# johannah/drqv2

Measured on AMD Instinct MI355X. Metric: agent updates/sec (batch=256, 9x84x84 obs), higher is better.
Workload: dtype f32; 1 GPU; cheetah_run batch_size=256/GPU (256 global) 9x84x84 u8 obs, A=6, feature_dim=50, hidden_dim=1024, fp32, use_tb=True; parallelism=dp1, global_batch=256

## Files before the change

drqv2_amd/_lib.py:

```python
import ctypes as C
import os

HERE = os.path.dirname(os.path.abspath(__file__))
LIB_PATH = os.path.join(HERE, "libdrqv2_hip.so")

c_float_p = C.c_void_p
c_u8_p = C.c_void_p
stream_t = C.c_void_p


class DrqStep(C.Structure):
    _fields_ = [
        ("B", C.c_int), ("global_B", C.c_int), ("C", C.c_int), ("A", C.c_int), ("F", C.c_int), ("H", C.c_int),
        ("obs", c_u8_p), ("next_obs", c_u8_p),
        ("action", c_float_p), ("reward", c_float_p), ("discount", c_float_p),
        ("shift_obs", c_float_p), ("shift_next", c_float_p),
        ("noise_critic", c_float_p), ("noise_actor", c_float_p),
        ("base_grid", c_float_p),
        ("params", c_float_p), ("grads", c_float_p), ("adam_m", c_float_p), ("adam_v", c_float_p),
        ("ws", c_float_p), ("ws_bytes", C.c_size_t),
        ("sums", c_float_p),
        ("lr", C.c_double), ("tau", C.c_double),
        ("std", C.c_float), ("clip", C.c_float),
        ("step_critic", C.c_long), ("step_enc", C.c_long), ("step_actor", C.c_long),
# ... 18 lines not shown
    "drq_conv1_aug_fwd": (I, [P, P, P, P, P, P, P, P, P, I, I, P]),
    "drq_conv1_aug_fwd_bf16": (I, [P, P, P, P, P, P, P, P, P, I, I, P]),
    "drq_conv1_aug_fwd_bf16_nhwc": (I, [P, P, P, P, P, P, P, P, P, I, I, P]),
    "drq_conv1_aug_fwd_indexed": (I, [P, P, P, P, P, P, P, P, P, P, P, I, I, P]),
    "drq_conv1_aug_fwd_frames": (I, [P, P, L, L, P, P, P, P, P, P, P, P, P, I, I, P]),
    "drq_conv1_aug_fwd_frames_bf16": (I, [P, P, L, L, P, P, P, P, P, P, P, P, P, I, I, P]),
    "drq_conv3x3_fwd": (I, [P, P, P, P, I, I, I, I, I, L, L, L, L, P]),
    "drq_conv3x3_dgrad": (I, [P, P, P, P, I, I, L, L, L, L, P]),
    "drq_conv3x3_fwd_wino": (I, [P, P, P, P, I, I, I, L, L, L, L, P]),
    "drq_conv3x3_dgrad_wino": (I, [P, P, P, P, I, I, L, L, L, L, P]),
    "drq_conv3x3_wgrad_wino": (I, [P, P, P, P, I, I, L, L, L, L, P, SZ, P]),
    "drq_conv3x3_wgrad": (I, [P, P, P, P, I, I, I, I, L, L, L, L, P, SZ, P]),
    "drq_conv3x3_wgrad_ws_bytes": (SZ, []),
    "drq_conv3x3_fwd_bf16": (I, [P, P, P, P, I, I, I, L, L, L, L, P]),
    "drq_conv3x3_dgrad_bf16": (I, [P, P, P, P, I, I, L, L, L, L, P]),
    "drq_conv3x3_wgrad_bf16": (I, [P, P, P, P, I, I, L, L, L, L, P, SZ, P]),
    "drq_conv3x3_fwd_bf16_nhwc": (I, [P, P, P, P, I, I, I, I, I, P]),
    "drq_conv3x3_dgrad_bf16_nhwc": (I, [P, P, P, P, I, I, I, I, L, L, L, L, P]),
    "drq_conv3x3_wgrad_bf16_nhwc": (I, [P, P, P, P, I, I, I, L, L, L, L, P, SZ, P]),
    "drq_gemm_f32": (I, [P, L, I, P, L, I, P, L, I, I, I, I, L, L, L, P, L, I, P, I, L, I, I, I, P, SZ, P]),
    "drq_gemm_batched_f32": (I, [I, P, L, I, P, L, I, P, L, I, I, I, P, I, P, I, P, I, I, I, P, SZ, P]),
    "drq_gemm_batched_bf16": (I, [I, P, L, I, P, L, I, P, L, I, I, I, P, I, P, I, P, I, I, P, SZ, P]),
    "drq_gemm_batched_partial": (I, [I, P, L, I, P, L, I, P, L, I, I, I, P, P, SZ, C.POINTER(I), P]),
    "drq_mlp_fwd": (I, [I, P, L, P, L, P, L, I, I, I, P, I, P, P, C.POINTER(I), P]),
    "drq_mlp_dgrad": (I, [I, P, L, P, L, P, L, I, I, I, P, I, P]),
    "drq_mlp_wgrad_dgrad": (I, [I, P, L, P, L, P, P, P, L, P, L, P, I, I, I, I, P]),
    "drq_ln_l1_fwd": (I, [I, P, P, P, P, P, P, P, P, P, P, P, P, P, P, P, P, P, I, I, I, L, P]),
    "drq_policy_out_l1_fwd": (I, [P, P, P, P, I, I, I, I, I, F, F, I, P, P, P, L, P, P, P, L, I, P, P, P, P]),
    "drq_qout_fwd": (I, [I, P, P, P, P, I, I, P]),
    "drq_qout_bwd": (I, [I, P, P, P, P, P, P, I, I, P]),
    "drq_ln_tanh_fwd_multi": (I, [I, P, I, P, P, P, P, P, P, I, I, P]),
    "drq_ln_tanh_fwd": (I, [P, I, P, P, P, I, P, P, I, I, P]),
    "drq_ln_tanh_fwd2": (I, [P, P, I, P, P, P, P, P, I, P, I, P, P, P, P, I, I, P]),
    "drq_ln_tanh_bwd": (I, [P, I, P, I, P, I, P, P, P, P, P, P, P, I, I, P]),
    "drq_colsum": (I, [P, L, L, P, L, I, I, I, P]),
    "drq_trunc_normal_sample": (I, [P, P, F, F, I, P, P, L, I, I, P]),
    "drq_copy_cols": (I, [P, I, P, L, I, I, P]),
    "drq_td_mse": (I, [P, P, P, P, P, P, P, P, P, I, F, P]),
    "drq_td_mse_w": (I, [P, P, P, P, P, P, P, P, P, P, P, I, F, P]),
    "drq_actor_loss": (I, [P, P, P, L, P, F, P, P, P, I, I, F, P]),
    "drq_actor_dmu": (I, [P, P, L, I, P, P, I, I, P]),
    "drq_actor_loss_bc": (I, [P, P, P, L, P, L, P, F, F, P, P, P, I, I, F, P]),
    "drq_qout_bwd_actor_bc": (I, [P, P, P, L, P, L, P, F, F, I, F, P, P, P, P, I, I, P]),
    "drq_actor_dmu_bc": (I, [P, P, L, I, P, P, L, P, L, F, P, I, I, P]),
    "drq_policy_out_bwd_bc": (I, [P, P, L, I, P, P, L, P, L, F, P, P, P, P, P, I, I, I, P, I, P]),
    "drq_adam_flat": (I, [P, P, P, P, L, D, L, F, P, D, P]),
# ... 92 lines not shown
```

drqv2_amd/csrc/gemm.hip:

```cpp
#include "common.h"
#include "internal.h"
#include "../../include/drqv2_hip.h"
#include <type_traits>

namespace {

constexpr int BK0 = 32;

constexpr int MAXB = 8;

struct Epilogue {
  const float* bias[MAXB];
  const float* aux[MAXB];
  float* rowsum[MAXB];
  int ldaux;
  int relu;
  int scatter_hw;
};

struct GemmArgs {
  const float* A[MAXB];
  const float* B[MAXB];
  float* C[MAXB];
  long lda, ldb, ldc;
// ... 81 lines not shown
    constexpr int KSTEP = 256 / BR;
    const bool rok = row0 + r < rows;
#pragma unroll
    for (int p = 0; p < BR * BK / 256; ++p)
      S[r * PK + kk0 + p * KSTEP] = (rok && k0 + kk0 + p * KSTEP < kend) ? reg[p] : 0.f;
  }
}

template <int BR, int BK>
__device__ __forceinline__ float tile_rowsum(const float (&reg)[BR * BK / 256], int row0, int rows, int k0, int kend,
                                             int tid) {
  const int r = tid % BR, kk0 = tid / BR;
  constexpr int KSTEP = 256 / BR;
  float s = 0.f;
  if (row0 + r < rows) {
#pragma unroll
    for (int p = 0; p < BR * BK / 256; ++p)
      if (k0 + kk0 + p * KSTEP < kend) s += reg[p];
  }
  return s;
}

template <int TM, int TN, bool A_KC, bool B_KC, bool V4, int BK = BK0, bool FULL = false>
__global__ __launch_bounds__(256) void gemm_kernel(GemmArgs g) {
  constexpr int PK = BK + 2;
  constexpr int BM = 32 * TM, BN = 32 * TN;
  constexpr int RA = BM * BK / 256, RB = BN * BK / 256;
  constexpr int D = (TM * TN == 1 && BK == 32) ? 4 : 2;
  __shared__ __attribute__((aligned(16))) float As[2][BM * PK];
  __shared__ __attribute__((aligned(16))) float Bs[2][BN * PK];

  const int tid = threadIdx.x;
  const int lane = tid & 63, wid = tid >> 6;
  const int wm = wid >> 1, wn = wid & 1;
  const int z = blockIdx.z;
  const int batch = z / g.splitk, ks = z - batch * g.splitk;
  const int m0 = blockIdx.y * BM, n0 = blockIdx.x * BN;
  const int kbeg = ks * g.kchunk;
  const int kend = min(g.K, kbeg + g.kchunk);
  const float* A = g.A[batch];
  const float* B = g.B[batch];

  float ra[D][RA], rb[D][RB];

  f32x4 acc[TM][TN];
#pragma unroll
  for (int i = 0; i < TM; ++i)
#pragma unroll
    for (int j = 0; j < TN; ++j) acc[i][j] = (f32x4){0.f, 0.f, 0.f, 0.f};

  const int arow = (wm * TM * 16 + (lane & 15)) * PK + (lane >> 4);
  const int brow = (wn * TN * 16 + (lane & 15)) * PK + (lane >> 4);
  const int nsteps = (kend - kbeg + BK - 1) / BK;

  auto fetch = [&](int t, float (&fa)[RA], float (&fb)[RB]) {
    const int tc = t < nsteps ? t : nsteps - 1;
    load_tile<BM, A_KC, V4, BK, FULL>(A, g.lda, m0, g.M, kbeg + tc * BK, kend, fa, tid);
    load_tile<BN, B_KC, V4, BK, FULL>(B, g.ldb, n0, g.N, kbeg + tc * BK, kend, fb, tid);
  };
  bool do_rs = false;
  if constexpr (!A_KC) do_rs = g.ep.rowsum[batch] != nullptr && blockIdx.x == 0;
  float rs = 0.f;
  if (nsteps > 0) {
    fetch(0, ra[0], rb[0]);
    if constexpr (!A_KC)
      if (do_rs) rs += tile_rowsum<BM, BK>(ra[0], m0, g.M, kbeg, kend, tid);
    store_tile<BM, A_KC, V4, BK, FULL>(As[0], ra[0], m0, g.M, kbeg, kend, tid);
    store_tile<BN, B_KC, V4, BK, FULL>(Bs[0], rb[0], n0, g.N, kbeg, kend, tid);
#pragma unroll
    for (int d = 1; d <= D; ++d) fetch(d, ra[d % D], rb[d % D]);
  }
  __syncthreads();
  auto step = [&](int t, auto sc) {
    constexpr int s = decltype(sc)::value;
    const float* as = As[s & 1];
    const float* bs = Bs[s & 1];
    float a[BK / 4][TM], b[BK / 4][TN];
#pragma unroll
    for (int kk = 0; kk < BK / 4; ++kk) {
#pragma unroll
      for (int i = 0; i < TM; ++i) a[kk][i] = as[arow + i * 16 * PK + kk * 4];
#pragma unroll
      for (int j = 0; j < TN; ++j) b[kk][j] = bs[brow + j * 16 * PK + kk * 4];
    }
// ... 87 lines not shown
#pragma unroll
    for (int j = 0; j < TN; ++j) {
      const int n = ncol0 + j * 16;
      long cbase = n;
      if (e.scatter_hw > 0) {
        const int hw = e.scatter_hw, hp = hw + 4;
        const int ch = n / (hw * hw);
        const int rr = n - ch * hw * hw;
        const int y = rr / hw, x = rr - y * hw;
        cbase = ((long)ch * hp + (y + 2)) * hp + (x + 2);
      }
#pragma unroll
      for (int r = 0; r < 4; ++r) {
        const int m = mrow0 + i * 16 + r;
        if (m < g.M && n < g.N) {
          float v = acc[i][j][r] + bv[j];
          if (e.relu) v = v > 0.f ? v : 0.f;
          v = av[i][j][r] > 0.f ? v : 0.f;
          if (e.scatter_hw > 0) c[(long)m * 32 * (e.scatter_hw + 4) * (e.scatter_hw + 4) + cbase] = v;
          else c[(long)m * g.ldc + cbase] = v;
        }
      }
    }
}

typedef __bf16 bf16x8_t __attribute__((ext_vector_type(8)));
typedef unsigned u32x4_t __attribute__((ext_vector_type(4)));

__device__ __forceinline__ unsigned pack_bf16_pair(float lo, float hi) {
  typedef __bf16 bf16x2_t __attribute__((ext_vector_type(2)));
  const bf16x2_t v = {(__bf16)lo, (__bf16)hi};
  return __builtin_bit_cast(unsigned, v);
}

constexpr int BF_BM = 64, BF_BK = 64, BF_PD = 36;

template <bool V4>
__device__ __forceinline__ void bf_load_kc(const float* P, long ld, int row0, int rows, int k0, int kend,
                                           float (&v)[16], int tid) {
  const int r = tid >> 2, kq = (tid & 3) * 16;
  const int row = row0 + r;
  if (V4 && row < rows && k0 + kq + 16 <= kend) {
    const f32x4* p = reinterpret_cast<const f32x4*>(P + (long)row * ld + k0 + kq);
#pragma unroll
    for (int i = 0; i < 4; ++i) {
      const f32x4 t = p[i];
// ... 202 lines not shown
    return v4 ? launch<TM, TN, true, false, true, BK>(g, st) : launch<TM, TN, true, false, false, BK>(g, st);
  if (!a_kc && !b_kc) return launch<TM, TN, false, false, false, BK>(g, st);
  return DRQ_EARG;
}

template <bool A_KC, bool B_KC>
int launch_bf16(const GemmArgs& g, bool v4, hipStream_t st) {
  const bool wide = g.N > 64 && g.N <= 128 && g.K >= 4096;
  const int bn = wide ? 2 * BF_BM : BF_BM;
  dim3 grid((g.N + bn - 1) / bn, (g.M + BF_BM - 1) / BF_BM, g.nbatch * g.splitk);
  if (wide) {
    if (v4) hipLaunchKernelGGL((gemm_bf16_kernel<A_KC, B_KC, true, 2>), grid, dim3(256), 0, st, g);
    else hipLaunchKernelGGL((gemm_bf16_kernel<A_KC, B_KC, false, 2>), grid, dim3(256), 0, st, g);
  } else if (v4) hipLaunchKernelGGL((gemm_bf16_kernel<A_KC, B_KC, true>), grid, dim3(256), 0, st, g);
  else hipLaunchKernelGGL((gemm_bf16_kernel<A_KC, B_KC, false>), grid, dim3(256), 0, st, g);
  DRQ_LAUNCH_CHECK();
  g_last_splitk = g.splitk;
  if (g.splitk > 1 && !g_leave_partials) {
    const long mn = (long)g.M * g.N;
    dim3 rg((unsigned)((mn + 255) / 256), g.nbatch);
    hipLaunchKernelGGL(splitk_reduce_kernel, rg, dim3(256), 0, st, g);
    DRQ_LAUNCH_CHECK();
  }
  return DRQ_OK;
}

}

int drq_gemm_batched_any(int bf16, int nbatch, const float* const* A, long lda, int a_kc, const float* const* B, long ldb,
                         int b_kc, float* const* C, long ldc, int M, int N, int K, const float* const* bias, int relu,
                         const float* const* aux, int ldaux, float* const* rowsum, int scatter_hw, int tile,
                         int splitk, float* ws, size_t ws_bytes, hipStream_t st) {
  if (!A || !B || !C || M <= 0 || N <= 0 || K <= 0 || nbatch <= 0 || nbatch > MAXB) return DRQ_EARG;
  for (int b = 0; b < nbatch; ++b)
    if (!A[b] || !B[b] || !C[b]) return DRQ_EARG;
  if (rowsum && a_kc) return DRQ_EARG;
  if (bf16) {
    if (!a_kc && b_kc) return DRQ_EARG;
    const int cus = drq_num_cus();
    const long tiles = (long)((M + 63) / 64) * ((N + 63) / 64) * nbatch;
    if (rowsum && splitk == 0 && tiles < 2L * cus && K >= 512) {
      for (int b = 0; b < nbatch; ++b)
        if (rowsum[b]) {
          const int rc = drq_colsum(A[b], lda, 0, rowsum[b], 0, K, M, 1, st);
          if (rc != DRQ_OK) return rc;
        }
// ... 24 lines not shown
    }
    g.lda = lda; g.ldb = ldb; g.ldc = ldc; g.M = M; g.N = N; g.K = K;
    g.nbatch = nbatch; g.splitk = splitk; g.kchunk = kchunk; g.part = ws;
    g.ep.ldaux = ldaux; g.ep.relu = relu; g.ep.scatter_hw = scatter_hw;
    if (a_kc && b_kc) return launch_bf16<true, true>(g, v4, st);
    if (a_kc && !b_kc) return launch_bf16<true, false>(g, v4, st);
    return launch_bf16<false, false>(g, v4, st);
  }
  if (nbatch == 1 && tile == 0 && splitk == 0 && N >= 4096 && N % 32 == 0 && !bias && !relu && a_kc && !b_kc &&
      K <= 128 && !rowsum) {
    const int rc =
        drq_skinny_dgrad(A[0], lda, B[0], ldb, C[0], ldc, M, N, K, aux ? aux[0] : nullptr, ldaux, scatter_hw, st);
    if (rc != DRQ_EARG) return rc;
  }
  if (nbatch == 1 && tile == 0 && splitk == 0 && scatter_hw == 0 && !a_kc && !b_kc && M <= 128 && N >= 4096 && !bias &&
      !relu && !aux) {
    const int rc = drq_trunk_wgrad(A[0], lda, B[0], ldb, C[0], ldc, M, N, K, rowsum ? rowsum[0] : nullptr, st);
    if (rc != DRQ_EARG) return rc;
  }
  if (tile == 0 && splitk == 0 && scatter_hw == 0) {
    const int rc = drq_gemm2(nbatch, A, lda, a_kc, B, ldb, b_kc, C, ldc, M, N, K, bias, relu, aux, ldaux, rowsum, st);
    if (rc != DRQ_EARG) return rc;
  }
  const int cus = drq_num_cus();
  const long t_big = (long)((M + 63) / 64) * ((N + 63) / 64) * nbatch;
  const long t_small = (long)((M + 31) / 32) * ((N + 31) / 32) * nbatch;
  if (tile == 0) tile = (t_big >= 2L * cus) ? 2 : 1;
  const long tiles = tile == 2 ? t_big : (tile >= 3 ? (t_big + t_small) / 2 : t_small);
  if (rowsum) splitk = 1;
  if (splitk == 0) {
    splitk = 1;
    if (tiles < 2L * cus && K >= 256) {
      splitk = (int)((3L * cus + tiles - 1) / tiles);
      const int maxs = K / 128;
      if (splitk > maxs) splitk = maxs;
      if (splitk < 1) splitk = 1;
    }
  }
  int kchunk = ((K + splitk - 1) / splitk + 63) / 64 * 64;
  splitk = (K + kchunk - 1) / kchunk;
  if (splitk > 1 && (!ws || (size_t)nbatch * splitk * M * N * sizeof(float) > ws_bytes)) return DRQ_EWS;
  GemmArgs g{};
  auto al16 = [](const void* p) { return ((uintptr_t)p & 15) == 0; };
  bool v4 = (K % 4 == 0) && (a_kc || b_kc);
  if (a_kc) v4 = v4 && lda % 4 == 0;
  if (b_kc) v4 = v4 && ldb % 4 == 0;
  for (int b = 0; b < nbatch; ++b) {
    g.A[b] = A[b]; g.B[b] = B[b]; g.C[b] = C[b];
    g.ep.bias[b] = bias ? bias[b] : nullptr;
    g.ep.aux[b] = aux ? aux[b] : nullptr;
    g.ep.rowsum[b] = rowsum ? rowsum[b] : nullptr;
    if (a_kc) v4 = v4 && al16(A[b]);
    if (b_kc) v4 = v4 && al16(B[b]);
  }
  g.lda = lda; g.ldb = ldb; g.ldc = ldc; g.M = M; g.N = N; g.K = K;
  g.nbatch = nbatch; g.splitk = splitk; g.kchunk = kchunk; g.part = ws;
  g.ep.ldaux = ldaux; g.ep.relu = relu; g.ep.scatter_hw = scatter_hw;
  if (tile == 3) return dispatch<2, 1>(g, a_kc, b_kc, v4, st);
  if (tile == 4) return dispatch<1, 2>(g, a_kc, b_kc, v4, st);
  if (tile == 5) return dispatch<1, 1, 64>(g, a_kc, b_kc, v4, st);
  if (tile == 6) return dispatch<2, 2, 64>(g, a_kc, b_kc, v4, st);
  return tile == 2 ? dispatch<2, 2>(g, a_kc, b_kc, v4, st) : dispatch<1, 1>(g, a_kc, b_kc, v4, st);
}

DRQ_API int drq_gemm_batched_f32(int nbatch, const float* const* A, long lda, int a_kc, const float* const* B, long ldb,
                         int b_kc, float* const* C, long ldc, int M, int N, int K, const float* const* bias, int relu,
                         const float* const* aux, int ldaux, float* const* rowsum, int scatter_hw, int tile,
                         int splitk, float* ws, size_t ws_bytes, drq_stream_t stream) {
  return drq_gemm_batched_any(0, nbatch, A, lda, a_kc, B, ldb, b_kc, C, ldc, M, N, K, bias, relu, aux, ldaux, rowsum,
                              scatter_hw, tile, splitk, ws, ws_bytes, (hipStream_t)stream);
}

DRQ_API int drq_gemm_batched_bf16(int nbatch, const float* const* A, long lda, int a_kc, const float* const* B, long ldb,
                          int b_kc, float* const* C, long ldc, int M, int N, int K, const float* const* bias, int relu,
                          const float* const* aux, int ldaux, float* const* rowsum, int scatter_hw, int splitk,
                          float* ws, size_t ws_bytes, drq_stream_t stream) {
  return drq_gemm_batched_any(1, nbatch, A, lda, a_kc, B, ldb, b_kc, C, ldc, M, N, K, bias, relu, aux, ldaux, rowsum,
                              scatter_hw, 0, splitk, ws, ws_bytes, (hipStream_t)stream);
}

// ... 4 lines not shown
  if (!bf16 && a_kc && b_kc && N <= 128 && K >= 4096 && ldc == N) {
    int sk = 1;
    const int rc = drq_trunk_fwd_partial(nbatch, A, lda, B, ldb, M, N, K, ws, ws_bytes, &sk, st);
    if (rc == DRQ_OK) {
      if (splitk_out) *splitk_out = sk;
      return DRQ_OK;
    }
    if (rc != DRQ_EARG) return rc;
  }
  g_leave_partials = true;
  g_last_splitk = 1;
  const int rc = drq_gemm_batched_any(bf16, nbatch, A, lda, a_kc, B, ldb, b_kc, C, ldc, M, N, K, bias, 0, nullptr, 0,
                                      nullptr, 0, bf16 ? 0 : 1, 0, ws, ws_bytes, st);
  g_leave_partials = false;
  if (splitk_out) *splitk_out = g_last_splitk;
  return rc;
}

DRQ_API int drq_gemm_batched_partial(int nbatch, const float* const* A, long lda, int a_kc, const float* const* B, long ldb,
                             int b_kc, float* const* C, long ldc, int M, int N, int K, const float* const* bias,
                             float* ws, size_t ws_bytes, int* splitk_out, drq_stream_t stream) {
  return drq_gemm_batched_partial_any(0, nbatch, A, lda, a_kc, B, ldb, b_kc, C, ldc, M, N, K, bias, ws, ws_bytes,
                                      splitk_out, (hipStream_t)stream);
}

DRQ_API int drq_gemm_f32(const float* A, long lda, int a_kc, const float* B, long ldb, int b_kc, float* C, long ldc,
                 int M, int N, int K, int nbatch, long a_bs, long b_bs, long c_bs, const float* bias, long bias_bs,
                 int relu, const float* aux, int ldaux, long aux_bs, int scatter_hw, int tile, int splitk,
                 float* ws, size_t ws_bytes, drq_stream_t stream) {
  if (!A || !B || !C || nbatch <= 0 || nbatch > MAXB) return DRQ_EARG;
  const float *Ap[MAXB], *Bp[MAXB], *bp[MAXB], *xp[MAXB];
  float* Cp[MAXB];
  for (int b = 0; b < nbatch; ++b) {
    Ap[b] = A + b * a_bs; Bp[b] = B + b * b_bs; Cp[b] = C + b * c_bs;
    bp[b] = bias ? bias + b * bias_bs : nullptr;
    xp[b] = aux ? aux + b * aux_bs : nullptr;
  }
  return drq_gemm_batched_f32(nbatch, Ap, lda, a_kc, Bp, ldb, b_kc, Cp, ldc, M, N, K, bias ? bp : nullptr, relu,
                              aux ? xp : nullptr, ldaux, nullptr, scatter_hw, tile, splitk, ws, ws_bytes, stream);
}
```

drqv2_amd/csrc/internal.h:

```cpp
#pragma once
#include "common.h"

int drq_ln_tanh_fwd_multi_ex(int n, const float* const* z, int ldz, const float* const* gamma,
                             const float* const* beta, float* const* out, const int* ldo, float* const* xhat,
                             float* const* rstd, int rows, int F, const float* const* tail, const int* tail_ld,
                             int tail_n, hipStream_t st);
int drq_ln_tanh_fwd_multi_part(int n, const float* const* z, int ldz, const float* const* gamma,
                               const float* const* beta, float* const* out, const int* ldo, float* const* xhat,
                               float* const* rstd, int rows, int F, const float* const* tail, const int* tail_ld,
                               int tail_n, const float* part, const float* const* bias, int splitk, hipStream_t st);
int drq_ln_tanh_bwd_part(const float* dh0, int ld0, const float* dh1, int ld1, const float* h, int ldh,
                         const float* xhat, const float* rstd, const float* gamma, float* dz, float* dln,
                         float* dgamma, float* dbeta, int rows, int F, const float* part, int splitk, int nprob,
                         int ldp, hipStream_t st);
int drq_ln_param_grad(const float* dln, const float* xhat, float* dgamma, float* dbeta, int rows, int F,
                      hipStream_t st);
int drq_qout_bwd_td(const float* tq1, const float* tq2, const float* q1, const float* q2, const float* reward,
                    const float* discount, float inv_global_B, float* sums, const float* const* h,
                    const float* const* w, float* const* dh, float* const* dw, float* const* db, int B, int H,
                    hipStream_t st);
int drq_qout_bwd_td_w(const float* tq1, const float* tq2, const float* q1, const float* q2, const float* reward,
                      const float* discount, const float* is_weight, float inv_global_B, float* sums, float* td_abs,
                      const float* const* h, const float* const* w, float* const* dh, float* const* dw,
                      float* const* db, int B, int H, hipStream_t st);
// ... 7 lines not shown
int drq_policy_out_bwd(const float* da1, const float* da2, long ld, int col0, const float* mu, const float* p2,
                       const float* w, float* dp2, float* dw, float* db, int B, int H, int A, const float* part,
                       int splitk, hipStream_t st);
int drq_actor_loss_ex(const float* q1, const float* q2, const float* a, long lda, const float* mu, float std,
                      float* dq1, float* dq2, float* sums, int B, int A, float inv_global_B, float* sums_host,
                      unsigned seq, hipStream_t st);
int drq_actor_loss_bc_ex(const float* q1, const float* q2, const float* a, long lda, const float* a_beh, long ldb,
                         const float* mu, float std, float alpha, float* dq1, float* dq2, float* sums, int B, int A,
                         float inv_global_B, float* sums_host, unsigned seq, hipStream_t st);
int drq_qout_bwd_actor_bc_ex(const float* q1, const float* q2, const float* act, long lda, const float* a_beh, long ldb,
                             const float* mu, float std, float alpha, int A, float inv_global_B, float* sums,
                             float* sums_host, unsigned seq, const float* const* h, const float* const* w,
                             float* const* dh, int B, int H, hipStream_t st);
int drq_adam_flat2(float* p0, const float* g0, float* m0, float* v0, long n0, long step0, float* p1, const float* g1,
                   float* m1, float* v1, long n1, long step1, double lr, float gscale, hipStream_t st);

int drq_gemm_batched_any(int bf16, int nbatch, const float* const* A, long lda, int a_kc, const float* const* B, long ldb,
                         int b_kc, float* const* C, long ldc, int M, int N, int K, const float* const* bias, int relu,
                         const float* const* aux, int ldaux, float* const* rowsum, int scatter_hw, int tile,
                         int splitk, float* ws, size_t ws_bytes, hipStream_t st);
int drq_gemm_batched_partial_any(int bf16, int nbatch, const float* const* A, long lda, int a_kc, const float* const* B,
                                 long ldb, int b_kc, float* const* C, long ldc, int M, int N, int K,
                                 const float* const* bias, float* ws, size_t ws_bytes, int* splitk_out, hipStream_t st);

int drq_skinny_dgrad(const float* dz, long lda, const float* w, long ldb, float* c, long ldc, int M, int N, int K,
                     const float* aux, int ldaux, int scatter_hw, hipStream_t st);

int drq_trunk_wgrad(const float* A, long lda, const float* B, long ldb, float* C, long ldc, int M, int N, int K,
                    float* rowsum, hipStream_t st);
int drq_trunk_wgrad_ln(const float* A, long lda, const float* B, long ldb, float* C, long ldc, int M, int N, int K,
                       float* rowsum, const float* ln_dln, const float* ln_xhat, float* ln_dgamma, float* ln_dbeta,
                       int ln_rows, int ln_F, hipStream_t st);
int drq_trunk_fwd_partial(int nbatch, const float* const* A, long lda, const float* const* B, long ldb, int M, int N,
                          int K, float* ws, size_t ws_bytes, int* splitk_out, hipStream_t st);
int drq_gemm2(int nbatch, const float* const* A, long lda, int a_kc, const float* const* B, long ldb, int b_kc,
              float* const* C, long ldc, int M, int N, int K, const float* const* bias, int relu,
              const float* const* aux, int ldaux, float* const* rowsum, hipStream_t st);
int drq_gemm2_wgrad_dgrad(int nbatch, const float* const* dy, long lddy, const float* const* x, long ldx,
                          float* const* dw, float* const* db, const float* const* w, long ldw, float* const* dx,
                          long lddx, const float* const* mask, int ldmask, int Brows, int Nout, int Kin, hipStream_t st);

int drq_gemm3_dgrad(int nbatch, const float* const* dy, long lddy, const float* const* w, long ldw, float* const* dx,
                    long lddx, int M, int N, int K, const float* const* mask, int ldmask, hipStream_t st);
int drq_gemm3_wgrad_dgrad(int nbatch, const float* const* dy, long lddy, const float* const* x, long ldx,
                          float* const* dw, float* const* db, const float* const* w, long ldw, float* const* dx,
                          long lddx, const float* const* mask, int ldmask, int Brows, int Nout, int Kin, hipStream_t st);
// ... 54 lines not shown
```

drqv2_amd/csrc/step.hip:

```cpp
#include "common.h"
#include "internal.h"
#include "../../include/drqv2_hip.h"

namespace {

constexpr long R = 32L * 35 * 35;
inline long al64(long x) { return (x + 63) & ~63L; }
inline long al512(long x) { return (x + 511) & ~511L; }

struct HeadOff {
  long trunk_w, trunk_b, ln_g, ln_b;
  long w[2][3], b[2][3];
};
enum { SEG_ENC, SEG_CRITIC, SEG_ACTOR, SEG_TARGET };
struct ParamLayout {
  long enc_w[4], enc_b[4];
  HeadOff critic, actor, target;
  long seg[8];
  long total;
  long flat[50];
  int nflat;
  long seg_beg(int net) const { return seg[2 * net]; }
  long seg_len(int net) const { return seg[2 * net + 1] - seg[2 * net]; }
};
// ... 189 lines not shown
    return drq_gemm_batched_any(bf16(), n, dy, lddy, 1, w, ldw, 0, dx, lddx, M, Nout, K, nullptr, 0, mask, ldmask, nullptr, 0,
                                0, 0, gemm_ws(), gemm_ws_bytes(), st);
  }
  int wgrad(int n, const float* const* dy, long lddy, const float* const* x, long ldx, float* const* dw,
            float* const* db, int Brows, int N, int K) const {
    const int prec = (bf16() && N <= 128 && K >= 4096 && Brows < 512) ? 0 : bf16();
    return drq_gemm_batched_any(prec, n, dy, lddy, 0, x, ldx, 0, dw, K, N, K, Brows, nullptr, 0, nullptr, 0, db, 0, 0, 0,
                                gemm_ws(), gemm_ws_bytes(), st);
  }
  bool ln_rides() const { return !bf16() && s->F <= 128 && (s->B == 128 || s->B == 256 || s->B == 512); }
  int trunk_wgrad(const float* dz, const float* feat, float* gw, float* gb, bool ride, const float* dln,
                  const float* xhat, float* dgamma, float* dbeta) const {
    const int B = s->B, F = s->F;
    if (ride) {
      const int rc = drq_trunk_wgrad_ln(dz, F, feat, R, gw, R, F, (int)R, B, gb, dln, xhat, dgamma, dbeta, B, F, st);
      if (rc != DRQ_EARG) return rc;
      const int rc2 = drq_ln_param_grad(dln, xhat, dgamma, dbeta, B, F, st);
      if (rc2 != 0) return rc2;
    }
    const float *dzp[1] = {dz}, *xp[1] = {feat};
    float *gwp[1] = {gw}, *gbp[1] = {gb};
    return wgrad(1, dzp, F, xp, R, gwp, gbp, B, F, (int)R);
  }
  int wgrad_dgrad(int n, const float* const* dy, long lddy, const float* const* x, long ldx, float* const* dw,
                  float* const* db, const float* const* w, long ldw, float* const* dx, long lddx,
                  const float* const* mask, int ldmask, int Brows, int N, int K) const {
    if (use_gemm3() && n >= 2) {
      const int rc = drq_gemm3_wgrad_dgrad(n, dy, lddy, x, ldx, dw, db, w, ldw, dx, lddx, mask, ldmask, Brows, N, K, st);
      if (rc != DRQ_EARG) return rc;
    }
    if (!bf16()) {
      const int rc = drq_gemm2_wgrad_dgrad(n, dy, lddy, x, ldx, dw, db, w, ldw, dx, lddx, mask, ldmask, Brows, N, K, st);
      if (rc != DRQ_EARG) return rc;
    }
    const int rc = wgrad(n, dy, lddy, x, ldx, dw, db, Brows, N, K);
    if (rc != 0) return rc;
    return dgrad(n, dy, lddy, w, ldw, dx, lddx, Brows, K, N, mask, ldmask);
  }
};

int encoder_forward(const Ctx& c, const float* x, int nb, float* a1, float* a2, float* a3, float* a4,
                    bool timed = false) {
  const ParamLayout& P = c.P;
  float* outs[4] = {a1, a2, a3, a4};
  const float* in = x ? x : a1;
  for (int l = x ? 0 : 1; l < 4; ++l) {
// ... 174 lines not shown
                *dc2c[2] = {dc2[0], dc2[1]}, *hac[2] = {c.ws(W_HA_C), c.ws(W_HA_C)};
    const float *w0[2] = {c.p(cr.w[0][0]), c.p(cr.w[1][0])}, *w1[2] = {c.p(cr.w[0][1]), c.p(cr.w[1][1])},
                *w2[2] = {c.p(cr.w[0][2]), c.p(cr.w[1][2])};
    float *gw0[2] = {c.g(cr.w[0][0]), c.g(cr.w[1][0])}, *gw1[2] = {c.g(cr.w[0][1]), c.g(cr.w[1][1])},
          *gw2[2] = {c.g(cr.w[0][2]), c.g(cr.w[1][2])};
    float *gb0[2] = {c.g(cr.b[0][0]), c.g(cr.b[1][0])}, *gb1[2] = {c.g(cr.b[0][1]), c.g(cr.b[1][1])},
          *gb2[2] = {c.g(cr.b[0][2]), c.g(cr.b[1][2])};
    if (c.qout_loss_fits_lds() && c.per()) {
      CK(drq_qout_bwd_td_w(c.ws(W_TQ), c.ws(W_TQ) + B, c.ws(W_Q), c.ws(W_Q) + B, s->reward, s->discount, c.is_weight,
                           invB, s->sums, c.td_abs, c2c, w2, dc2, gw2, gb2, B, H, st));
    } else if (c.qout_loss_fits_lds()) {
      CK(drq_qout_bwd_td(c.ws(W_TQ), c.ws(W_TQ) + B, c.ws(W_Q), c.ws(W_Q) + B, s->reward, s->discount, invB, s->sums,
                         c2c, w2, dc2, gw2, gb2, B, H, st));
    } else {
      if (c.per())
        CK(drq_td_mse_w(c.ws(W_TQ), c.ws(W_TQ) + B, c.ws(W_Q), c.ws(W_Q) + B, s->reward, s->discount, c.is_weight,
                        c.ws(W_DQ), c.ws(W_DQ) + B, c.td_abs, s->sums, B, invB, st));
      else
        CK(drq_td_mse(c.ws(W_TQ), c.ws(W_TQ) + B, c.ws(W_Q), c.ws(W_Q) + B, s->reward, s->discount, c.ws(W_DQ),
                      c.ws(W_DQ) + B, s->sums, B, invB, st));
      CK(drq_qout_bwd(2, dq, c2c, w2, dc2, gw2, gb2, B, H, st));
    }
    CK(c.wgrad_dgrad(2, dc2c, H, c1c, H, gw1, gb1, w1, H, dc1, H, c1c, H, B, H, H));
    CK(c.wgrad(2, dc1c, H, hac, FA, gw0, gb0, B, H, FA));
    CK(drq_gemm_batched_partial_any(c.bf16(), 2, dc1c, H, 1, w0, FA, 0, dha, FA, B, FA, H, nullptr, c.gemm_ws(), c.gemm_ws_bytes(),
                                &sk_dha, st));
  }
  const bool ride = c.ln_rides();
  CK(drq_ln_tanh_bwd_part(c.ws(W_DHA), FA, c.ws(W_DHA) + (long)B * FA, FA, c.ws(W_HA_C), FA, c.ws(W_XHAT_C),
                          c.ws(W_RSTD_C), c.p(cr.ln_g), c.ws(W_DZ_C), c.ws(W_DLN), ride ? nullptr : c.g(cr.ln_g),
                          ride ? nullptr : c.g(cr.ln_b), B, F, sk_dha > 1 ? c.gemm_ws() : nullptr, sk_dha, 2, FA, st));
  {
    const float *dz[1] = {c.ws(W_DZ_C)}, *w[1] = {c.p(cr.trunk_w)}, *mk[1] = {feat_obs};
    float* dy4[1] = {c.ws(W_DY4)};
    CK(c.trunk_wgrad(c.ws(W_DZ_C), feat_obs, c.g(cr.trunk_w), c.g(cr.trunk_b), ride, c.ws(W_DLN), c.ws(W_XHAT_C),
                     c.g(cr.ln_g), c.g(cr.ln_b)));
    CK(drq_gemm_batched_any(0, 1, dz, F, 1, w, R, 0, dy4, 0, B, (int)R, F, nullptr, 0, mk, (int)R, nullptr, 35, 0, 0,
                            c.gemm_ws(), c.gemm_ws_bytes(), st));
  }

  return 0;
}

int phase_conv_backward(const Ctx& c) {
  const DrqStep* s = c.s;
  const ParamLayout& P = c.P;
  const int B = s->B, C = s->C;
  hipStream_t st = c.st;
  const int dyid[4] = {W_DY1, W_DY2, W_DY3, W_DY4};
// ... 172 lines not shown
  else if (!fused_head)
    CK(drq_actor_dmu(c.ws(W_DA), c.ws(W_DA) + (long)B * A, A, 0, c.ws(W_MU_O), c.ws(W_DPRE), B, A, st));

  int sk_dh = 1;
  {
    const float *dpre[1] = {c.ws(W_DPRE)}, *p1[1] = {c.ws(W_P1)}, *p2[1] = {c.ws(W_P2)}, *h[1] = {c.ws(W_HROWS)};
    float *dp1[1] = {c.ws(W_DP1)}, *dp2[1] = {c.ws(W_DP2)}, *dh[1] = {c.ws(W_DH_A)};
    const float *dp1c[1] = {dp1[0]}, *dp2c[1] = {dp2[0]};
    const float *w0[1] = {c.p(ac.w[0][0])}, *w1[1] = {c.p(ac.w[0][1])}, *w2[1] = {c.p(ac.w[0][2])};
    float *gw0[1] = {c.g(ac.w[0][0])}, *gw1[1] = {c.g(ac.w[0][1])}, *gw2[1] = {c.g(ac.w[0][2])};
    float *gb0[1] = {c.g(ac.b[0][0])}, *gb1[1] = {c.g(ac.b[0][1])}, *gb2[1] = {c.g(ac.b[0][2])};
    if (fused_head && c.bc()) {
      CK(drq_policy_out_bwd_bc(c.ws(W_DA), c.ws(W_DA) + (long)B * A, A, 0, c.ws(W_MU_O), c.ws(W_HA_C2) + F, FA, c.a_beh(),
                               FA, c.bc_scale(), p2[0], w2[0], dp2[0], gw2[0], gb2[0], B, H, A,
                               sk_da > 1 ? c.gemm_ws() : nullptr, sk_da, st));
    } else if (fused_head) {
      CK(drq_policy_out_bwd(c.ws(W_DA), c.ws(W_DA) + (long)B * A, A, 0, c.ws(W_MU_O), p2[0], w2[0], dp2[0], gw2[0],
                            gb2[0], B, H, A, sk_da > 1 ? c.gemm_ws() : nullptr, sk_da, st));
    } else {
      CK(c.wgrad(1, dpre, A, p2, H, gw2, gb2, B, A, H));
      CK(c.dgrad(1, dpre, A, w2, H, dp2, H, B, H, A, p2, H));
    }
    CK(c.wgrad_dgrad(1, dp2c, H, p1, H, gw1, gb1, w1, H, dp1, H, p1, H, B, H, H));
    CK(c.wgrad(1, dp1c, H, h, F, gw0, gb0, B, H, F));
    CK(drq_gemm_batched_partial_any(c.bf16(), 1, dp1c, H, 1, w0, F, 0, dh, F, B, F, H, nullptr, c.gemm_ws(), c.gemm_ws_bytes(), &sk_dh,
                                st));
  }
  const bool ride = c.ln_rides();
  CK(drq_ln_tanh_bwd_part(c.ws(W_DH_A), F, nullptr, 0, c.ws(W_HROWS), F, c.ws(W_XHAT_A), c.ws(W_RSTD_A), c.p(ac.ln_g),
                          c.ws(W_DZ_A), c.ws(W_DLN), ride ? nullptr : c.g(ac.ln_g), ride ? nullptr : c.g(ac.ln_b), B, F,
                          sk_dh > 1 ? c.gemm_ws() : nullptr, sk_dh, 1, F, st));
  CK(c.trunk_wgrad(c.ws(W_DZ_A), feat_obs, c.g(ac.trunk_w), c.g(ac.trunk_b), ride, c.ws(W_DLN), c.ws(W_XHAT_A),
                   c.g(ac.ln_g), c.g(ac.ln_b)));
  return 0;
}

int phase_both_opt(const Ctx& c) {
  const DrqStep* s = c.s;
  const ParamLayout& P = c.P;
  const long e = P.seg_beg(SEG_ENC), a = P.seg_beg(SEG_ACTOR);
  return drq_adam_flat2(c.p(e), c.g(e), s->adam_m + e, s->adam_v + e, P.seg_len(SEG_ENC), s->step_enc, c.p(a), c.g(a),
                        s->adam_m + a, s->adam_v + a, P.seg_len(SEG_ACTOR), s->step_actor, s->lr, s->gscale, c.st);
}

bool runs(int phase, int part) {
  switch (phase) {
    case DRQ_PHASE_ALL: return (part >= DRQ_PHASE_ENCODE && part <= DRQ_PHASE_ACTOR_BACKWARD) || part == DRQ_PHASE_OPT;
    case DRQ_PHASE_CRITIC: return part >= DRQ_PHASE_ENCODE && part <= DRQ_PHASE_CONV_BACKWARD;
    case DRQ_PHASE_ACTOR: return part == DRQ_PHASE_ACTOR_FORWARD || part == DRQ_PHASE_ACTOR_BACKWARD;
// ... 155 lines not shown
```

include/drqv2_hip.h:

```cpp
#ifndef DRQV2_HIP_H
#define DRQV2_HIP_H
#include <stddef.h>
#include <stdint.h>

#ifdef __cplusplus
extern "C" {
#endif

typedef void* drq_stream_t;

#define DRQ_OK 0
#define DRQ_EARG (-1)
#define DRQ_EWS (-2)

int drq_abi_version(void);

int drq_aug_fwd(const uint8_t* obs, const float* shift_xy, const float* base_grid, float* out, int n, int c,
                int hw, int pad, int fuse_norm, drq_stream_t stream);
int drq_aug_fwd_f32(const float* x, const float* shift_xy, const float* base_grid, float* out, int n, int c,
                    int hw, int pad, drq_stream_t stream);

int drq_conv1_aug_fwd(const uint8_t* obs, const float* shift, const uint8_t* obs1, const float* shift1,
                      const float* base_grid, const float* w, const float* bias, float* xaug, float* y, int n,
                      int n_store, drq_stream_t stream);
// ... 43 lines not shown
                                drq_stream_t stream);
int drq_conv3x3_wgrad_bf16_nhwc(const void* x_nhwc, const void* dy, float* dw, float* db, int nb, int hin, int dy_nhwc,
                                long dy_bs, long dy_cs, long dy_rs, long dy_off, float* ws, size_t ws_bytes,
                                drq_stream_t stream);

int drq_gemm_f32(const float* A, long lda, int a_kc, const float* B, long ldb, int b_kc, float* C, long ldc,
                 int M, int N, int K, int nbatch, long a_bs, long b_bs, long c_bs, const float* bias, long bias_bs,
                 int relu, const float* aux, int ldaux, long aux_bs, int scatter_hw, int tile, int splitk,
                 float* ws, size_t ws_bytes, drq_stream_t stream);

int drq_gemm_batched_f32(int nbatch, const float* const* A, long lda, int a_kc, const float* const* B, long ldb,
                         int b_kc, float* const* C, long ldc, int M, int N, int K, const float* const* bias, int relu,
                         const float* const* aux, int ldaux, float* const* rowsum, int scatter_hw, int tile,
                         int splitk, float* ws, size_t ws_bytes, drq_stream_t stream);

int drq_gemm_batched_bf16(int nbatch, const float* const* A, long lda, int a_kc, const float* const* B, long ldb,
                          int b_kc, float* const* C, long ldc, int M, int N, int K, const float* const* bias, int relu,
                          const float* const* aux, int ldaux, float* const* rowsum, int scatter_hw, int splitk,
                          float* ws, size_t ws_bytes, drq_stream_t stream);

int drq_gemm_batched_partial(int nbatch, const float* const* A, long lda, int a_kc, const float* const* B, long ldb,
                             int b_kc, float* const* C, long ldc, int M, int N, int K, const float* const* bias,
                             float* ws, size_t ws_bytes, int* splitk_out, drq_stream_t stream);

int drq_mlp_fwd(int nbatch, const float* const* x, long ldx, const float* const* w, long ldw, float* const* y,
                long ldy, int M, int N, int K, const float* const* bias, int relu, const float* const* qw,
                float* const* qpart, int* nq_out, drq_stream_t stream);
int drq_mlp_dgrad(int nbatch, const float* const* dy, long lddy, const float* const* w, long ldw, float* const* dx,
                  long lddx, int M, int N, int K, const float* const* mask, int ldmask, drq_stream_t stream);
int drq_mlp_wgrad_dgrad(int nbatch, const float* const* dy, long lddy, const float* const* x, long ldx,
                        float* const* dw, float* const* db, const float* const* w, long ldw, float* const* dx,
                        long lddx, const float* const* mask, int ldmask, int Brows, int Nout, int Kin,
                        drq_stream_t stream);

int drq_ln_l1_fwd(int njobs, const float* const* part, const float* const* z, const float* const* bias,
                  const float* const* gamma, const float* const* beta, float* const* out, const int* ldo,
                  float* const* xhat, float* const* rstd, const float* const* tail, const int* tail_ld,
                  const int* tail_n, const int* rows, const int* nheads, const float* const* w, const float* const* b,
                  float* const* y, int F, int H, int splitk, long slab, drq_stream_t stream);
int drq_policy_out_l1_fwd(const float* p2, const float* w3, const float* b3, float* p3, int rows, int srow0, int H, int A,
                          int F, float std, float clip, int use_clip, const float* noise_hi, float* mu_hi, float* ha_hi,
                          long lda_hi, const float* noise_lo, float* mu_lo, float* ha_lo, long lda_lo, int nheads,
                          const float* const* w, const float* const* b, float* const* y, drq_stream_t stream);

int drq_qout_fwd(int nz, const float* const* h, const float* const* w, const float* const* b, float* const* q, int B,
                 int H, drq_stream_t stream);
// ... 111 lines not shown
  float* adam_m;
  float* adam_v;
  float* ws;
  size_t ws_bytes;
  float* sums;
  double lr, tau;
  float std, clip;
  long step_critic, step_enc, step_actor;
  float gscale;
  drq_stream_t stream;
  float* sums_host;
  int store_aug_next;
  int bf16;
  void* const* timing_events;
  int timing_n;
  const int64_t* obs_index;
  const int64_t* next_obs_index;
  int flags;
} DrqStep;
#define DRQ_STEP_NO_ROW_FUSION 1
#define DRQ_STEP_NO_GEMM3 2
#define DRQ_STEP_BF16_FP32_ACTS 4
#define DRQ_STEP_BF16_FP32_GRADS 8

int drq_param_layout(int C, int A, int F, int H, long* out, int cap);
#define DRQ_PARAM_LAYOUT_LEN 59

size_t drq_step_ws_bytes(int B, int C, int A, int F, int H);
long drq_step_ws_offset(int B, int C, int A, int F, int H, int buffer_id);
enum {
  DRQ_WS_AUG = 0, DRQ_WS_ACT1, DRQ_WS_ACT2, DRQ_WS_ACT3, DRQ_WS_FEAT, DRQ_WS_Z_NEXT, DRQ_WS_Z_OBS,
  DRQ_WS_HA_T, DRQ_WS_HA_C, DRQ_WS_H_AN, DRQ_WS_H_AO, DRQ_WS_Q, DRQ_WS_TQ, DRQ_WS_DQ, DRQ_WS_MU_O,
  DRQ_WS_DY4, DRQ_WS_DY3, DRQ_WS_DY2, DRQ_WS_DY1, DRQ_WS_DZ_C, DRQ_WS_DZ_A, DRQ_WS_HA_C2,
  DRQ_WS_P1, DRQ_WS_P2,
  DRQ_WS_C1, DRQ_WS_C2,
  DRQ_WS_NBUF_PUBLIC
};

enum {
  DRQ_PHASE_ALL = -1, DRQ_PHASE_CRITIC = 0, DRQ_PHASE_ACTOR = 1, DRQ_PHASE_OPT = 2,
  DRQ_PHASE_ENCODE = 3, DRQ_PHASE_CRITIC_HEADS = 4, DRQ_PHASE_CONV_BACKWARD = 5, DRQ_PHASE_ACTOR_FORWARD = 6,
  DRQ_PHASE_ACTOR_BACKWARD = 7, DRQ_PHASE_ENCODER_OPT = 8, DRQ_PHASE_ACTOR_OPT = 9,
  DRQ_PHASE_CRITIC_OPT = 10, DRQ_PHASE_ACTOR_LOSS = 11, DRQ_PHASE_POLYAK = 12, DRQ_PHASE_REDRAW = 13
};
int drq_update_phase(const DrqStep* s, int phase);
int drq_update_phase_bc(const DrqStep* s, int phase, float bc_alpha);
// ... 18 lines not shown
```

Baseline: 974.5 updates/s.

## Fuse first-layer wgrad and dgrad GEMMs into one paired-grid launch

Pulls the fp32 GEMM body out into a device function and adds a paired kernel. The kernel splits one flat 1D grid between the weight-gradient GEMM and the data-gradient GEMM of the first MLP layer, in both the critic and actor backward passes. The intent is to replace two kernel launches with one and let blocks from both small GEMMs run on the GPU at the same time, filling more CUs. If the shapes don't qualify (e.g. all dimensions multiples of 32, wide K, or the planner picks a non-small tile), it falls back to the old two-launch path, and a new step flag can switch it off. The cost is a shared kernel whose register and LDS budget must suit both GEMM variants.

```diff
diff --git a/drqv2_amd/_lib.py b/drqv2_amd/_lib.py
--- a/drqv2_amd/_lib.py
+++ b/drqv2_amd/_lib.py
@@ -64,6 +64,7 @@
     "drq_gemm_batched_f32": (I, [I, P, L, I, P, L, I, P, L, I, I, I, P, I, P, I, P, I, I, I, P, SZ, P]),
     "drq_gemm_batched_bf16": (I, [I, P, L, I, P, L, I, P, L, I, I, I, P, I, P, I, P, I, I, P, SZ, P]),
     "drq_gemm_batched_partial": (I, [I, P, L, I, P, L, I, P, L, I, I, I, P, P, SZ, C.POINTER(I), P]),
+    "drq_gemm_wgrad_dgrad_partial": (I, [I, P, L, P, L, P, P, P, L, P, L, I, I, I, P, SZ, C.POINTER(I), P]),
     "drq_mlp_fwd": (I, [I, P, L, P, L, P, L, I, I, I, P, I, P, P, C.POINTER(I), P]),
     "drq_mlp_dgrad": (I, [I, P, L, P, L, P, L, I, I, I, P, I, P]),
     "drq_mlp_wgrad_dgrad": (I, [I, P, L, P, L, P, P, P, L, P, L, P, I, I, I, I, P]),
diff --git a/drqv2_amd/csrc/gemm.hip b/drqv2_amd/csrc/gemm.hip
--- a/drqv2_amd/csrc/gemm.hip
+++ b/drqv2_amd/csrc/gemm.hip
@@ -1,5 +1,6 @@
 #include "common.h"
 #include "internal.h"
+#include "pair_grid.h"
 #include "../../include/drqv2_hip.h"
 #include <type_traits>
 
@@ -127,20 +128,18 @@
 }
 
 template <int TM, int TN, bool A_KC, bool B_KC, bool V4, int BK = BK0, bool FULL = false>
-__global__ __launch_bounds__(256) void gemm_kernel(GemmArgs g) {
+__device__ __forceinline__ void gemm_body(const GemmArgs& g, const int bx, const int by, const int z,
+                                          float (&As)[2][32 * TM * (BK + 2)], float (&Bs)[2][32 * TN * (BK + 2)]) {
   constexpr int PK = BK + 2;
   constexpr int BM = 32 * TM, BN = 32 * TN;
   constexpr int RA = BM * BK / 256, RB = BN * BK / 256;
   constexpr int D = (TM * TN == 1 && BK == 32) ? 4 : 2;
-  __shared__ __attribute__((aligned(16))) float As[2][BM * PK];
-  __shared__ __attribute__((aligned(16))) float Bs[2][BN * PK];
 
   const int tid = threadIdx.x;
   const int lane = tid & 63, wid = tid >> 6;
   const int wm = wid >> 1, wn = wid & 1;
-  const int z = blockIdx.z;
   const int batch = z / g.splitk, ks = z - batch * g.splitk;
-  const int m0 = blockIdx.y * BM, n0 = blockIdx.x * BN;
+  const int m0 = by * BM, n0 = bx * BN;
   const int kbeg = ks * g.kchunk;
   const int kend = min(g.K, kbeg + g.kchunk);
   const float* A = g.A[batch];
@@ -164,7 +163,7 @@
     load_tile<BN, B_KC, V4, BK, FULL>(B, g.ldb, n0, g.N, kbeg + tc * BK, kend, fb, tid);
   };
   bool do_rs = false;
-  if constexpr (!A_KC) do_rs = g.ep.rowsum[batch] != nullptr && blockIdx.x == 0;
+  if constexpr (!A_KC) do_rs = g.ep.rowsum[batch] != nullptr && bx == 0;
   float rs = 0.f;
   if (nsteps > 0) {
     fetch(0, ra[0], rb[0]);
@@ -298,6 +297,22 @@
         }
       }
     }
+}
+
+template <int TM, int TN, bool A_KC, bool B_KC, bool V4, int BK = BK0, bool FULL = false>
+__global__ __launch_bounds__(256) void gemm_kernel(GemmArgs g) {
+  __shared__ __attribute__((aligned(16))) float As[2][32 * TM * (BK + 2)];
+  __shared__ __attribute__((aligned(16))) float Bs[2][32 * TN * (BK + 2)];
+  gemm_body<TM, TN, A_KC, B_KC, V4, BK, FULL>(g, (int)blockIdx.x, (int)blockIdx.y, (int)blockIdx.z, As, Bs);
+}
+
+template <bool V4>
+__global__ __launch_bounds__(256) void gemm_pair_kernel(GemmArgs gw, GemmArgs gd, PairGrid pg) {
+  __shared__ __attribute__((aligned(16))) float As[2][32 * (BK0 + 2)];
+  __shared__ __attribute__((aligned(16))) float Bs[2][32 * (BK0 + 2)];
+  const PairBlock b = pair_block(pg, (int)blockIdx.x);
+  if (b.set == 0) gemm_body<1, 1, false, false, false>(gw, b.x, b.y, b.z, As, Bs);
+  else gemm_body<1, 1, true, false, V4>(gd, b.x, b.y, b.z, As, Bs);
 }
 
 typedef __bf16 bf16x8_t __attribute__((ext_vector_type(8)));
@@ -546,6 +561,46 @@
     hipLaunchKernelGGL(splitk_reduce_kernel, rg, dim3(256), 0, st, g);
     DRQ_LAUNCH_CHECK();
   }
+  return DRQ_OK;
+}
+
+int plan_f32(GemmArgs& g, int& tile, bool& v4, int nbatch, const float* const* A, long lda, int a_kc,
+             const float* const* B, long ldb, int b_kc, float* const* C, long ldc, int M, int N, int K,
+             const float* const* bias, int relu, const float* const* aux, int ldaux, float* const* rowsum,
+             int scatter_hw, int splitk, float* ws, size_t ws_bytes) {
+  const int cus = drq_num_cus();
+  const long t_big = (long)((M + 63) / 64) * ((N + 63) / 64) * nbatch;
+  const long t_small = (long)((M + 31) / 32) * ((N + 31) / 32) * nbatch;
+  if (tile == 0) tile = (t_big >= 2L * cus) ? 2 : 1;
+  const long tiles = tile == 2 ? t_big : (tile >= 3 ? (t_big + t_small) / 2 : t_small);
+  if (rowsum) splitk = 1;
+  if (splitk == 0) {
+    splitk = 1;
+    if (tiles < 2L * cus && K >= 256) {
+      splitk = (int)((3L * cus + tiles - 1) / tiles);
+      const int maxs = K / 128;
+      if (splitk > maxs) splitk = maxs;
+      if (splitk < 1) splitk = 1;
+    }
+  }
+  int kchunk = ((K + splitk - 1) / splitk + 63) / 64 * 64;
+  splitk = (K + kchunk - 1) / kchunk;
+  if (splitk > 1 && (!ws || (size_t)nbatch * splitk * M * N * sizeof(float) > ws_bytes)) return DRQ_EWS;
+  auto al16 = [](const void* p) { return ((uintptr_t)p & 15) == 0; };
+  v4 = (K % 4 == 0) && (a_kc || b_kc);
+  if (a_kc) v4 = v4 && lda % 4 == 0;
+  if (b_kc) v4 = v4 && ldb % 4 == 0;
+  for (int b = 0; b < nbatch; ++b) {
+    g.A[b] = A[b]; g.B[b] = B[b]; g.C[b] = C[b];
+    g.ep.bias[b] = bias ? bias[b] : nullptr;
+    g.ep.aux[b] = aux ? aux[b] : nullptr;
+    g.ep.rowsum[b] = rowsum ? rowsum[b] : nullptr;
+    if (a_kc) v4 = v4 && al16(A[b]);
+    if (b_kc) v4 = v4 && al16(B[b]);
+  }
+  g.lda = lda; g.ldb = ldb; g.ldc = ldc; g.M = M; g.N = N; g.K = K;
+  g.nbatch = nbatch; g.splitk = splitk; g.kchunk = kchunk; g.part = ws;
+  g.ep.ldaux = ldaux; g.ep.relu = relu; g.ep.scatter_hw = scatter_hw;
   return DRQ_OK;
 }
 
@@ -616,40 +671,11 @@
     const int rc = drq_gemm2(nbatch, A, lda, a_kc, B, ldb, b_kc, C, ldc, M, N, K, bias, relu, aux, ldaux, rowsum, st);
     if (rc != DRQ_EARG) return rc;
   }
-  const int cus = drq_num_cus();
-  const long t_big = (long)((M + 63) / 64) * ((N + 63) / 64) * nbatch;
-  const long t_small = (long)((M + 31) / 32) * ((N + 31) / 32) * nbatch;
-  if (tile == 0) tile = (t_big >= 2L * cus) ? 2 : 1;
-  const long tiles = tile == 2 ? t_big : (tile >= 3 ? (t_big + t_small) / 2 : t_small);
-  if (rowsum) splitk = 1;
-  if (splitk == 0) {
-    splitk = 1;
-    if (tiles < 2L * cus && K >= 256) {
-      splitk = (int)((3L * cus + tiles - 1) / tiles);
-      const int maxs = K / 128;
-      if (splitk > maxs) splitk = maxs;
-      if (splitk < 1) splitk = 1;
-    }
-  }
-  int kchunk = ((K + splitk - 1) / splitk + 63) / 64 * 64;
-  splitk = (K + kchunk - 1) / kchunk;
-  if (splitk > 1 && (!ws || (size_t)nbatch * splitk * M * N * sizeof(float) > ws_bytes)) return DRQ_EWS;
   GemmArgs g{};
-  auto al16 = [](const void* p) { return ((uintptr_t)p & 15) == 0; };
-  bool v4 = (K % 4 == 0) && (a_kc || b_kc);
-  if (a_kc) v4 = v4 && lda % 4 == 0;
-  if (b_kc) v4 = v4 && ldb % 4 == 0;
-  for (int b = 0; b < nbatch; ++b) {
-    g.A[b] = A[b]; g.B[b] = B[b]; g.C[b] = C[b];
-    g.ep.bias[b] = bias ? bias[b] : nullptr;
-    g.ep.aux[b] = aux ? aux[b] : nullptr;
-    g.ep.rowsum[b] = rowsum ? rowsum[b] : nullptr;
-    if (a_kc) v4 = v4 && al16(A[b]);
-    if (b_kc) v4 = v4 && al16(B[b]);
-  }
-  g.lda = lda; g.ldb = ldb; g.ldc = ldc; g.M = M; g.N = N; g.K = K;
-  g.nbatch = nbatch; g.splitk = splitk; g.kchunk = kchunk; g.part = ws;
-  g.ep.ldaux = ldaux; g.ep.relu = relu; g.ep.scatter_hw = scatter_hw;
+  bool v4 = false;
+  const int rc = plan_f32(g, tile, v4, nbatch, A, lda, a_kc, B, ldb, b_kc, C, ldc, M, N, K, bias, relu, aux, ldaux, rowsum,
+                          scatter_hw, splitk, ws, ws_bytes);
+  if (rc != DRQ_OK) return rc;
   if (tile == 3) return dispatch<2, 1>(g, a_kc, b_kc, v4, st);
   if (tile == 4) return dispatch<1, 2>(g, a_kc, b_kc, v4, st);
   if (tile == 5) return dispatch<1, 1, 64>(g, a_kc, b_kc, v4, st);
@@ -700,6 +726,46 @@
                              float* ws, size_t ws_bytes, int* splitk_out, drq_stream_t stream) {
   return drq_gemm_batched_partial_any(0, nbatch, A, lda, a_kc, B, ldb, b_kc, C, ldc, M, N, K, bias, ws, ws_bytes,
                                       splitk_out, (hipStream_t)stream);
+}
+
+int drq_gemm_wgrad_dgrad_partial_any(int bf16, int nbatch, const float* const* dy, long lddy, const float* const* x,
+                                     long ldx, float* const* dw, float* const* db, const float* const* w, long ldw,
+                                     float* const* dx, long lddx, int Brows, int Nout, int Kin, float* ws,
+                                     size_t ws_bytes, int* splitk_out, hipStream_t st) {
+  if (bf16 || !dy || !x || !dw || !db || !w || !dx || nbatch <= 0 || nbatch > MAXB || Brows <= 0 || Nout <= 0 || Kin <= 0)
+    return DRQ_EARG;
+  for (int b = 0; b < nbatch; ++b)
+    if (!dy[b] || !x[b] || !dw[b] || !db[b] || !w[b] || !dx[b]) return DRQ_EARG;
+  if (Brows % 32 == 0 && Nout % 32 == 0 && Kin % 32 == 0) return DRQ_EARG;
+  if (Kin >= 4096) return DRQ_EARG;
+  GemmArgs gw{}, gd{};
+  int tw = 0, td = 1;
+  bool v4w = false, v4d = false;
+  int rc = plan_f32(gw, tw, v4w, nbatch, dy, lddy, 0, x, ldx, 0, dw, Kin, Nout, Kin, Brows, nullptr, 0, nullptr, 0, db, 0, 0,
+                    ws, ws_bytes);
+  if (rc != DRQ_OK) return rc;
+  if (tw != 1 || gw.splitk != 1) return DRQ_EARG;
+  rc = plan_f32(gd, td, v4d, nbatch, dy, lddy, 1, w, ldw, 0, dx, lddx, Brows, Kin, Nout, nullptr, 0, nullptr, 0, nullptr, 0,
+                0, ws, ws_bytes);
+  if (rc != DRQ_OK) return rc;
+  PairGrid pg{};
+  const long total = pair_grid(pg, (gw.N + 31) / 32, (gw.M + 31) / 32, nbatch, (gd.N + 31) / 32, (gd.M + 31) / 32,
+                               nbatch * gd.splitk);
+  if (total < 0) return DRQ_EARG;
+  const dim3 grid((unsigned)total);
+  if (v4d) hipLaunchKernelGGL((gemm_pair_kernel<true>), grid, dim3(256), 0, st, gw, gd, pg);
+  else hipLaunchKernelGGL((gemm_pair_kernel<false>), grid, dim3(256), 0, st, gw, gd, pg);
+  DRQ_LAUNCH_CHECK();
+  if (splitk_out) *splitk_out = gd.splitk;
+  return DRQ_OK;
+}
+
+DRQ_API int drq_gemm_wgrad_dgrad_partial(int nbatch, const float* const* dy, long lddy, const float* const* x, long ldx,
+                                         float* const* dw, float* const* db, const float* const* w, long ldw,
+                                         float* const* dx, long lddx, int Brows, int Nout, int Kin, float* ws,
+                                         size_t ws_bytes, int* splitk_out, drq_stream_t stream) {
+  return drq_gemm_wgrad_dgrad_partial_any(0, nbatch, dy, lddy, x, ldx, dw, db, w, ldw, dx, lddx, Brows, Nout, Kin, ws,
+                                          ws_bytes, splitk_out, (hipStream_t)stream);
 }
 
 DRQ_API int drq_gemm_f32(const float* A, long lda, int a_kc, const float* B, long ldb, int b_kc, float* C, long ldc,
diff --git a/drqv2_amd/csrc/internal.h b/drqv2_amd/csrc/internal.h
--- a/drqv2_amd/csrc/internal.h
+++ b/drqv2_amd/csrc/internal.h
@@ -53,6 +53,10 @@
 int drq_gemm_batched_partial_any(int bf16, int nbatch, const float* const* A, long lda, int a_kc, const float* const* B,
                                  long ldb, int b_kc, float* const* C, long ldc, int M, int N, int K,
                                  const float* const* bias, float* ws, size_t ws_bytes, int* splitk_out, hipStream_t st);
+int drq_gemm_wgrad_dgrad_partial_any(int bf16, int nbatch, const float* const* dy, long lddy, const float* const* x,
+                                     long ldx, float* const* dw, float* const* db, const float* const* w, long ldw,
+                                     float* const* dx, long lddx, int Brows, int Nout, int Kin, float* ws,
+                                     size_t ws_bytes, int* splitk_out, hipStream_t st);
 
 int drq_skinny_dgrad(const float* dz, long lda, const float* w, long ldb, float* c, long ldc, int M, int N, int K,
                      const float* aux, int ldaux, int scatter_hw, hipStream_t st);
diff --git a/drqv2_amd/csrc/pair_grid.h b/drqv2_amd/csrc/pair_grid.h
--- /dev/null
+++ b/drqv2_amd/csrc/pair_grid.h
@@ -0,0 +1,30 @@
+#pragma once
+#if defined(__HIPCC__)
+#define DRQ_HD __host__ __device__
+#else
+#define DRQ_HD
+#endif
+
+struct PairGrid {
+  int n0;
+  int x0, y0;
+  int x1, y1;
+};
+struct PairBlock {
+  int set, x, y, z;
+};
+
+inline long pair_grid(PairGrid& pg, int x0, int y0, int z0, int x1, int y1, int z1) {
+  if (x0 <= 0 || y0 <= 0 || z0 <= 0 || x1 <= 0 || y1 <= 0 || z1 <= 0) return -1;
+  const long n0 = (long)x0 * y0 * z0, n1 = (long)x1 * y1 * z1;
+  if (n0 / z0 / y0 != x0 || n1 / z1 / y1 != x1 || n0 >= (1L << 31) || n1 >= (1L << 31) || n0 + n1 >= (1L << 31)) return -1;
+  pg.n0 = (int)n0; pg.x0 = x0; pg.y0 = y0; pg.x1 = x1; pg.y1 = y1;
+  return n0 + n1;
+}
+
+DRQ_HD inline PairBlock pair_block(const PairGrid& pg, int i) {
+  const int set = i < pg.n0 ? 0 : 1;
+  const int j = set ? i - pg.n0 : i, gx = set ? pg.x1 : pg.x0, gy = set ? pg.y1 : pg.y0;
+  const int r = j / gx;
+  return PairBlock{set, j - r * gx, r % gy, r / gy};
+}
diff --git a/drqv2_amd/csrc/step.hip b/drqv2_amd/csrc/step.hip
--- a/drqv2_amd/csrc/step.hip
+++ b/drqv2_amd/csrc/step.hip
@@ -235,6 +235,20 @@
     float *gwp[1] = {gw}, *gbp[1] = {gb};
     return wgrad(1, dzp, F, xp, R, gwp, gbp, B, F, (int)R);
   }
+  bool pairs() const { return !(s->flags & DRQ_STEP_NO_PAIRS); }
+  int wgrad_dgrad_partial(int n, const float* const* dy, long lddy, const float* const* x, long ldx, float* const* dw,
+                          float* const* db, const float* const* w, long ldw, float* const* dx, long lddx, int Brows, int N,
+                          int K, int* sk) const {
+    if (pairs()) {
+      const int rc = drq_gemm_wgrad_dgrad_partial_any(bf16(), n, dy, lddy, x, ldx, dw, db, w, ldw, dx, lddx, Brows, N, K,
+                                                      gemm_ws(), gemm_ws_bytes(), sk, st);
+      if (rc != DRQ_EARG) return rc;
+    }
+    const int rc = wgrad(n, dy, lddy, x, ldx, dw, db, Brows, N, K);
+    if (rc != 0) return rc;
+    return drq_gemm_batched_partial_any(bf16(), n, dy, lddy, 1, w, ldw, 0, dx, lddx, Brows, K, N, nullptr, gemm_ws(),
+                                        gemm_ws_bytes(), sk, st);
+  }
   int wgrad_dgrad(int n, const float* const* dy, long lddy, const float* const* x, long ldx, float* const* dw,
                   float* const* db, const float* const* w, long ldw, float* const* dx, long lddx,
                   const float* const* mask, int ldmask, int Brows, int N, int K) const {
@@ -455,9 +469,7 @@
       CK(drq_qout_bwd(2, dq, c2c, w2, dc2, gw2, gb2, B, H, st));
     }
     CK(c.wgrad_dgrad(2, dc2c, H, c1c, H, gw1, gb1, w1, H, dc1, H, c1c, H, B, H, H));
-    CK(c.wgrad(2, dc1c, H, hac, FA, gw0, gb0, B, H, FA));
-    CK(drq_gemm_batched_partial_any(c.bf16(), 2, dc1c, H, 1, w0, FA, 0, dha, FA, B, FA, H, nullptr, c.gemm_ws(), c.gemm_ws_bytes(),
-                                &sk_dha, st));
+    CK(c.wgrad_dgrad_partial(2, dc1c, H, hac, FA, gw0, gb0, w0, FA, dha, FA, B, H, FA, &sk_dha));
   }
   const bool ride = c.ln_rides();
   CK(drq_ln_tanh_bwd_part(c.ws(W_DHA), FA, c.ws(W_DHA) + (long)B * FA, FA, c.ws(W_HA_C), FA, c.ws(W_XHAT_C),
@@ -676,9 +688,7 @@
       CK(c.dgrad(1, dpre, A, w2, H, dp2, H, B, H, A, p2, H));
     }
     CK(c.wgrad_dgrad(1, dp2c, H, p1, H, gw1, gb1, w1, H, dp1, H, p1, H, B, H, H));
-    CK(c.wgrad(1, dp1c, H, h, F, gw0, gb0, B, H, F));
-    CK(drq_gemm_batched_partial_any(c.bf16(), 1, dp1c, H, 1, w0, F, 0, dh, F, B, F, H, nullptr, c.gemm_ws(), c.gemm_ws_bytes(), &sk_dh,
-                                st));
+    CK(c.wgrad_dgrad_partial(1, dp1c, H, h, F, gw0, gb0, w0, F, dh, F, B, H, F, &sk_dh));
   }
   const bool ride = c.ln_rides();
   CK(drq_ln_tanh_bwd_part(c.ws(W_DH_A), F, nullptr, 0, c.ws(W_HROWS), F, c.ws(W_XHAT_A), c.ws(W_RSTD_A), c.p(ac.ln_g),
diff --git a/include/drqv2_hip.h b/include/drqv2_hip.h
--- a/include/drqv2_hip.h
+++ b/include/drqv2_hip.h
@@ -89,6 +89,11 @@
 int drq_gemm_batched_partial(int nbatch, const float* const* A, long lda, int a_kc, const float* const* B, long ldb,
                              int b_kc, float* const* C, long ldc, int M, int N, int K, const float* const* bias,
                              float* ws, size_t ws_bytes, int* splitk_out, drq_stream_t stream);
+
+int drq_gemm_wgrad_dgrad_partial(int nbatch, const float* const* dy, long lddy, const float* const* x, long ldx,
+                                 float* const* dw, float* const* db, const float* const* w, long ldw, float* const* dx,
+                                 long lddx, int Brows, int Nout, int Kin, float* ws, size_t ws_bytes, int* splitk_out,
+                                 drq_stream_t stream);
 
 int drq_mlp_fwd(int nbatch, const float* const* x, long ldx, const float* const* w, long ldw, float* const* y,
                 long ldy, int M, int N, int K, const float* const* bias, int relu, const float* const* qw,
@@ -246,6 +251,7 @@
 #define DRQ_STEP_NO_GEMM3 2
 #define DRQ_STEP_BF16_FP32_ACTS 4
 #define DRQ_STEP_BF16_FP32_GRADS 8
+#define DRQ_STEP_NO_PAIRS 16
 
 int drq_param_layout(int C, int A, int F, int H, long* out, int cap);
 #define DRQ_PARAM_LAYOUT_LEN 59
```

After: 982.7 updates/s, median of 6. About the same (+0.8%).
